# mitschabaude/montgomery

Hardware: AMD Instinct MI355X
Metric: BLS12-377 G1 MSM throughput (higher is better)
Workload: dtype u32

## Files before the change

montgomery_amd/csrc/msm_sort.hip:

```cpp
#include "msm_internal.h"

using namespace msm;
using namespace msmi;

namespace msmi {

void sort_kernel_attributes() {
  HIPCHK(hipFuncSetAttribute((const void*)k_hist, hipFuncAttributeMaxDynamicSharedMemorySize, 128 * 1024));
  HIPCHK(hipFuncSetAttribute((const void*)k_scatter_lds, hipFuncAttributeMaxDynamicSharedMemorySize, 128 * 1024));
  HIPCHK(hipFuncSetAttribute((const void*)k_bin_split, hipFuncAttributeMaxDynamicSharedMemorySize, (int)bin_split_lds(1u << BS_MAX_AB)));
  HIPCHK(hipFuncSetAttribute((const void*)k_bin_pairs, hipFuncAttributeMaxDynamicSharedMemorySize, (int)bin_pairs_lds(1u << BS_MAX_FB)));
  HIPCHK(hipFuncSetAttribute((const void*)k_bin_slots, hipFuncAttributeMaxDynamicSharedMemorySize, (int)bin_slots_lds(1u << BS_MAX_FB)));
  const int dig_lds = 16 * (1 << BS_MAX_AB) * 4;
#define MSM_DIGITS_ATTR(ID, CV) HIPCHK(hipFuncSetAttribute((const void*)k_digits<CV>, hipFuncAttributeMaxDynamicSharedMemorySize, dig_lds));
  MSM_W_CURVES(MSM_DIGITS_ATTR)
#undef MSM_DIGITS_ATTR
  HIPCHK(hipFuncSetAttribute((const void*)te::k_te_digits, hipFuncAttributeMaxDynamicSharedMemorySize, dig_lds));
#define MSM_NARROW_ATTR(W)                                                                                                    \
  HIPCHK(hipFuncSetAttribute((const void*)k_digits_narrow<W>, hipFuncAttributeMaxDynamicSharedMemorySize, dig_lds));          \
  HIPCHK(hipFuncSetAttribute((const void*)k_te_digits_narrow<W>, hipFuncAttributeMaxDynamicSharedMemorySize, dig_lds));
  MSM_NARROW_WIDTHS(MSM_NARROW_ATTR)
#undef MSM_NARROW_ATTR
}

// ... 124 lines not shown
  } else if (radix && cuts) {
    if (kc > 16) throw MsmFail{MSM_ERR_INTERNAL, "more than 16 windows in a radix-split group"};
    for (int kk = 0; kk < kc; kk++) { ws.ab[kk] = (uint8_t)(cbits - (int)RX_FINE_BITS); ws.fb[kk] = (uint8_t)RX_FINE_BITS; }
  }
  const uint32_t Hn = radix ? 1u << (cbits - (int)RX_FINE_BITS) : 1u;
  const uint32_t V = (uint32_t)kc * (bin_split ? hb : Hn);
  uint32_t sortB = 1;
  uint64_t chunk = two_n, pps = n;
  if (bin_split) {
    const uint64_t mult = 4;
    sortB = (uint32_t)std::max<uint64_t>(1, std::min<uint64_t>((uint64_t)mult * ctx->n_cu, n / 4096));
    const uint64_t max_pps = (1ull << BS_SPAN_LOG) / (te ? 1 : 2);
    sortB = (uint32_t)std::max<uint64_t>(sortB, (n + max_pps - 1) / max_pps);
    pps = (n + sortB - 1) / sortB;
    chunk = (te ? 1 : 2) * pps;
    if (consume) {
      if (share->sortB != sortB || share->pps != pps || share->chunk != chunk || share->hb < hb)
        throw MsmFail{MSM_ERR_INTERNAL, "shared digits do not match the group's sort geometry"};
      hb = share->hb;
    } else {
      ctx->ensure(w.block_hist, (size_t)kc_d * sortB * hb * 4 + 64);
    }
  } else {
    const uint64_t mult = two_n >= (1ull << 27) ? 8 : two_n >= (1ull << 24) ? 4 : 2;
    uint64_t want = std::max<uint64_t>(1, (mult * ctx->n_cu + kc - 1) / kc);
    uint64_t maxb = std::max<uint64_t>(1, two_n / 8192);
    sortB = (uint32_t)std::min<uint64_t>(want, maxb);
    chunk = (two_n + sortB - 1) / sortB;
    if (!produce) ctx->ensure(w.block_hist, (size_t)kc * sortB * L * 4 + 64);
  }
  uint32_t* d_bin_start = nullptr;
  uint32_t *d_extra_first = nullptr, *d_mp_first = nullptr, *d_part_pair_off = nullptr;
  uint32_t part_len = 0, part_grid = 0;
  bool will_chunk = false;
  {
    const int chunk_rows_log = ctx->chunk_rows_log;
    const uint64_t table_rows = pl.tables ? (uint64_t)kc_d * n : n;
    const bool want_chunks = bin_split && !te && pl.c >= 18 && table_rows > (1ull << chunk_rows_log);
    will_chunk = bin_split && want_chunks && !te && logG >= 2;
  }
  if (produce && !bin_split && !digits_only) return;
  if (produce) ctx->ensure(w.dig, n_entries * 4);
  if (share && !share->produce && !bin_split) throw MsmFail{MSM_ERR_INTERNAL, "shared digits for a group that does not take the bin split"};
  const uint32_t* dig_p = consume ? share->dig + (uint64_t)(k_lo - share->k_lo) * two_n_d : (const uint32_t*)w.dig.p;
  uint32_t* hist_p = consume ? share->hist + (uint64_t)(k_lo - share->k_lo) * sortB * hb : (uint32_t*)w.block_hist.p;

  if (consume) HIPCHK(hipStreamWaitEvent(s, share->ready, 0));
  HIPCHK(hipEventRecord(w.ev[0], s));
  if (pl.nar.width) {
    if (!consume) narrow_digits(ctx, w, d_scalars, n, pl, k_lo, kc_d, bin_split, radix, sortB, pps, hb, ws, digits_only);
  } else if (pl.batch) {
    if (((bin_split || radix) && !digits_only) || k_lo != 0 || kc_d != pl.batch * pl.K) throw MsmFail{MSM_ERR_INTERNAL, "a batch group outside the one-level sort"};
    const uint32_t grid = (uint32_t)((n + 255) / 256);
    if (te)
      hipLaunchKernelGGL(te::k_te_digits_batch, dim3(grid), dim3(256), 0, s, (uint32_t*)w.dig.p, pl.batch_sc, (uint32_t)pl.batch,
                         (uint32_t)n, pl.c, pl.K, pl.strict ? 1 : 0, (uint32_t*)ctx->errflag.p);
    else
      W_LAUNCH(ctx, k_digits_batch, dim3(grid), dim3(256), 0, s, (uint32_t*)w.dig.p, pl.batch_sc, (uint32_t)pl.batch, (uint32_t)n, pl.c,
               pl.K, (pl.no_glv ? 0 : 1) | (pl.fold ? 2 : 0), pl.strict ? 1 : 0, (uint32_t*)ctx->errflag.p);
  } else if (!consume) {
    const uint32_t grid = bin_split ? sortB : (uint32_t)((n + 255) / 256);
    const uint32_t per = bin_split ? (uint32_t)pps : 256u;
    uint32_t* hist = bin_split ? (uint32_t*)w.block_hist.p : nullptr;
    const size_t lds = bin_split ? (size_t)kc_d * hb * 4 : 0;
    WinSplit ws_d = ws;
    if (pl.tables) for (int kk = 0; kk < 16; kk++) ws_d.fb[kk] = ws.fb[0];
    const uint32_t threads = bin_split ? 1024u : 256u;
    if (te)
      hipLaunchKernelGGL(te::k_te_digits, dim3(grid), dim3(threads), lds, s, (uint32_t*)w.dig.p, d_scalars, (uint32_t)n, pl.c, pl.K,
                         k_lo, kc_d, pl.strict ? 1 : 0, (uint32_t*)ctx->errflag.p, per, hist, hb, pack_fine_bits(ws_d), pl.b_lo, pl.b_n, pl.bt_lo, pl.bt_n);
    else
      W_LAUNCH(ctx, k_digits, dim3(grid), dim3(threads), lds, s, (uint32_t*)w.dig.p, d_scalars, (uint32_t)n, pl.c, pl.K, k_lo, kc_d,
                         (pl.no_glv ? 0 : 1) | (pl.fold ? 2 : 0), pl.strict ? 1 : 0, (uint32_t*)ctx->errflag.p, per, hist, hb, pack_fine_bits(ws_d), pl.b_lo, pl.b_n, pl.bt_lo, pl.bt_n);
  }
  if (produce) {
    share->k_lo = k_lo;
    share->dig = (const uint32_t*)w.dig.p;
    share->hist = (uint32_t*)w.block_hist.p;
    share->hb = hb;
    share->sortB = sortB;
    share->pps = pps;
    share->chunk = chunk;
    HIPCHK(hipEventRecord(share->ready, s));
    share->valid = true;
    return;
  }
  HIPCHK(hipEventRecord(w.ev[1], s));
  if (!bin_split) {
    hipLaunchKernelGGL(k_hist, dim3(sortB, kc), dim3(SORT_THREADS), (size_t)L * 4, s, (uint32_t*)w.block_hist.p,
                       (const uint32_t*)w.dig.p, two_n, chunk, L);
    hipLaunchKernelGGL(k_colscan, dim3((uint32_t)((nb + 255) / 256)), dim3(256), 0, s, (uint32_t*)w.block_hist.p,
                       (uint32_t*)w.counts.p, sortB, L, (uint32_t)kc);
  } else {
    ctx->ensure(w.part, ((size_t)2 * V + 2) * 4);
    uint32_t* d_bin_tot = (uint32_t*)w.part.p;
    d_bin_start = d_bin_tot + V;
    ctx->ensure(w.rec, n_entries * 8);
    hipLaunchKernelGGL(k_slice_scan, dim3((hb + 31) / 32, kc), dim3(1024), 0, s, hist_p, d_bin_tot,
                       pl.tables ? sortB * (uint32_t)kc_d : sortB, hb, (uint32_t)kc);
    part_len = (uint32_t)std::max<uint64_t>(1u << 16, ((2 * n_entries / V + BP_TILE - 1) / BP_TILE) * BP_TILE);
    part_grid = V + V / 2 + 1;
    ctx->ensure(w.parts, ((size_t)2 * (V + 1) + (V + 2)) * 4);
    d_extra_first = (uint32_t*)w.parts.p;
    d_mp_first = d_extra_first + (V + 1);
    d_part_pair_off = d_mp_first + (V + 1);
    PartTables ptab{d_extra_first, d_mp_first, d_part_pair_off, hb, part_len, {}};
    for (int kk = 0; kk < 16; kk++) ptab.fb[kk] = ws.fb[kk];
    hipLaunchKernelGGL(k_vscan, dim3(1), dim3(SCAN_THREADS), 0, s, d_bin_start, (const uint32_t*)d_bin_tot, V, (uint32_t*)w.info.p, ptab);
    const uint32_t per_block = (uint32_t)std::min<uint64_t>(std::min<uint64_t>(sortB, std::max<uint64_t>(1, (1ull << BS_SPAN_LOG) / chunk)),
                                                            std::max<uint64_t>(1, (2 * (uint64_t)BS_TILE + chunk - 1) / chunk));
    hipLaunchKernelGGL(k_bin_split, dim3((sortB + per_block - 1) / per_block, kc_d), dim3(BS_THREADS), bin_split_lds(hb), s, (uint2*)w.rec.p,
                       (const uint32_t*)d_bin_start, (const uint32_t*)hist_p, dig_p, two_n_d, chunk, hb, ws,
                       pl.tables ? 1u : 0u, sortB, per_block);
    bool spans_all = true;
    for (int kk = 0; kk < kc; kk++) spans_all &= (1u << ws.ab[kk]) == hb && (int)ws.ab[kk] + (int)ws.fb[kk] == cbits;
    if (!spans_all) HIPCHK(hipMemsetAsync(w.counts.p, 0, nb * 4, s));
    ctx->ensure(w.sub, (size_t)(V + 2) * nbmax * 4);
    hipLaunchKernelGGL(k_bin_count, dim3(part_grid), dim3(BC_THREADS), (size_t)nbmax * 4, s, (uint32_t*)w.counts.p, (const uint32_t*)d_bin_start,
                       (const uint2*)w.rec.p, hb, L, ws, (uint32_t*)w.info.p, V, (const uint32_t*)d_extra_first, (const uint32_t*)d_mp_first,
                       part_len, (uint32_t*)w.sub.p, nbmax);
    hipLaunchKernelGGL(k_part_scan, dim3(V), dim3(PSC_THREADS), 0, s, (uint32_t*)w.counts.p, (uint32_t*)w.sub.p, d_part_pair_off,
                       (const uint32_t*)d_extra_first, (const uint32_t*)d_mp_first, hb, L, nbmax, ws, (uint32_t*)w.info.p,
                       will_chunk ? 1u : 0u);
  }
  scan_bucket_sizes(ctx, w, nb, logG, !bin_split);
  const uint32_t* round1_slots = nullptr;
  const uint32_t* round1_dest = nullptr;
  uint64_t rec_y_off = 0;
  bool chunked = will_chunk;
  const uint64_t parts_extra = will_chunk ? std::min<uint64_t>(n_entries, (uint64_t)V * nbmax) : 0;
  const uint64_t slots_bound = n_entries + parts_extra + (((uint64_t)1 << logG) - 1) * std::min<uint64_t>(nb, n_entries);
  auto launch_bin_pass = [&](uint64_t slots_cap) {
    if (chunked) {
      const uint64_t pairs_cap = slots_cap / 2 + 1;
      ctx->ensure(w.slots2, pairs_cap * 8);
      ctx->ensure(w.dest, pairs_cap * 4);
      rec_y_off = (pairs_cap * 64 + 255) & ~(uint64_t)255;
      ctx->ensure(w.rows1, 2 * rec_y_off + 256);
      hipLaunchKernelGGL(k_bin_pairs, dim3(part_grid), dim3(BP_THREADS), bin_pairs_lds(nbmax), s, (uint2*)w.slots2.p, (uint32_t*)w.dest.p,
                         (const uint2*)w.rec.p, (const uint32_t*)d_bin_start, (const uint32_t*)w.cursor.p, hb, L, nbmax, ws, V,
                         (const uint32_t*)d_extra_first, (const uint32_t*)d_mp_first, part_len, (const uint32_t*)w.sub.p,
                         (const uint32_t*)d_part_pair_off);
      round1_slots = (const uint32_t*)w.slots2.p;
      round1_dest = (const uint32_t*)w.dest.p;
    } else {
      ctx->ensure(w.slots, std::max<uint64_t>(slots_cap, 2) * 4);
      HIPCHK(hipMemsetAsync(w.slots.p, 0xFF, std::max<uint64_t>(slots_cap, 2) * 4, s));
      round1_slots = (const uint32_t*)w.slots.p;
      hipLaunchKernelGGL(k_bin_slots, dim3(part_grid), dim3(BP_THREADS), bin_slots_lds(nbmax), s, (uint32_t*)w.slots.p,
                         (const uint2*)w.rec.p, (const uint32_t*)d_bin_start, (const uint32_t*)w.cursor.p, hb, L, nbmax, ws, V,
                         (const uint32_t*)d_extra_first, (const uint32_t*)d_mp_first, part_len, (const uint32_t*)w.sub.p);
    }
  };
  if (bin_split) launch_bin_pass(slots_bound);
  const ScanTotals tot = read_scan_totals(w, logG);
  const int RT = tot.RT;
  const uint64_t total_slots = tot.total_slots;
  const uint32_t max_bucket = tot.max_bucket;
  st.n_pairs_algo += tot.algo_pairs;
  st.max_bucket = std::max<uint64_t>(st.max_bucket, max_bucket);
  if (total_slots > slots_bound) throw MsmFail{MSM_ERR_INTERNAL, "the padded slots exceed their bound"};
  if (bin_split && chunked && total_slots < 2) {
    chunked = false;
    round1_dest = nullptr;
    rec_y_off = 0;
    launch_bin_pass(2);
  }
  if (!bin_split) {
    ctx->ensure(w.slots, std::max<uint64_t>(total_slots, 2) * 4);
    HIPCHK(hipMemsetAsync(w.slots.p, 0xFF, std::max<uint64_t>(total_slots, 2) * 4, s));
    round1_slots = (const uint32_t*)w.slots.p;
    const bool heavy = radix && max_bucket >= (1u << 16) && (uint64_t)max_bucket * Hn >= 16 * two_n;
    if (radix && !heavy) {
      ctx->ensure(w.part, ((size_t)kc * sortB * Hn + 2 * (size_t)V + 2) * 4);
      uint32_t* d_blk_off = (uint32_t*)w.part.p;
      uint32_t* d_vtot = d_blk_off + (size_t)kc * sortB * Hn;
      uint32_t* d_vstart = d_vtot + V;
      ctx->ensure(w.dig2, n_entries * 4);
      ctx->ensure(w.idx2, n_entries * 4);
      const uint64_t co = (uint64_t)kc * (sortB + 1) * Hn;
      hipLaunchKernelGGL(k_coarse_offsets, dim3((uint32_t)((co + 255) / 256)), dim3(256), 0, s, d_blk_off, d_vtot,
                         (const uint32_t*)w.block_hist.p, (const uint32_t*)w.counts.p, sortB, L, Hn, (uint32_t)kc);
      hipLaunchKernelGGL(k_vscan, dim3(1), dim3(SCAN_THREADS), 0, s, d_vstart, (const uint32_t*)d_vtot, V, (uint32_t*)nullptr, PartTables{});
      hipLaunchKernelGGL(k_radix_coarse, dim3(sortB, kc), dim3(RX_THREADS), 0, s, (uint32_t*)w.dig2.p, (uint32_t*)w.idx2.p,
// ... 23 lines not shown
```

montgomery_amd/csrc/sort_kernels.h:

```cpp
#pragma once
#include "msm_kernels.h"

namespace msm {


constexpr int SCAN_THREADS = 1024;
constexpr int SCAN_ITEMS = 4;

__device__ __forceinline__ void lds_barrier() {
#if defined(__HIP_DEVICE_COMPILE__)
  asm volatile("s_waitcnt lgkmcnt(0)\n\ts_barrier" ::: "memory");
#endif
}

template <bool LDS_ONLY = false>
MSM_DEV uint32_t block_excl_scan(uint32_t v, uint32_t* lds_wave, uint32_t& total) {
  uint32_t x = v;
  const int lane = threadIdx.x & 63, wave = threadIdx.x >> 6;
#pragma unroll
  for (int d = 1; d < 64; d <<= 1) {
    uint32_t y = __shfl_up(x, d, 64);
    if (lane >= d) x += y;
  }
  if (LDS_ONLY) lds_barrier(); else __syncthreads();
// ... 492 lines not shown
      uint32_t v[8];
#pragma unroll
      for (int i = 0; i < 8; i++) v[i] = p[(uint64_t)(b + i) * L];
#pragma unroll
      for (int i = 0; i < 8; i++) sum += v[i];
    }
    for (; b < b1; b++) sum += p[(uint64_t)b * L];
  }
  part[r][c] = sum;
  __syncthreads();
  uint32_t run = 0;
  for (uint32_t q = 0; q < r; q++) run += part[q][c];
  if (live) {
    uint32_t b = b0;
    for (; b + 8 <= b1; b += 8) {
      uint32_t v[8];
#pragma unroll
      for (int i = 0; i < 8; i++) v[i] = p[(uint64_t)(b + i) * L];
#pragma unroll
      for (int i = 0; i < 8; i++) { p[(uint64_t)(b + i) * L] = run; run += v[i]; }
    }
    for (; b < b1; b++) {
      const uint32_t v = p[(uint64_t)b * L];
      p[(uint64_t)b * L] = run;
      run += v;
    }
    if (r == 31) totals[(uint64_t)kk * L + l] = run;
  }
}
#endif

constexpr uint32_t BS_MAX_AB = 11, BS_MAX_FB = 12;
constexpr uint32_t BS_SPAN_LOG = 17;
inline size_t bin_split_lds(uint32_t hb) { return (size_t)BS_TILE * 4 + (size_t)3 * hb * 4 + 64 * 4; }

__global__ void __launch_bounds__(BS_THREADS) k_bin_split(uint2* rec, const uint32_t* bin_start, const uint32_t* slice_off,
                                                          const uint32_t* dig, uint64_t two_n, uint64_t chunk, uint32_t hb, WinSplit ws,
                                                          uint32_t merged, uint32_t SBd, uint32_t g)
#ifndef MSM_SORT_TU
    ;
#else
{
  extern __shared__ uint32_t lds_bs[];
  uint32_t* stage = lds_bs;
  uint32_t* t_cnt = stage + BS_TILE;
  uint32_t* t_start = t_cnt + hb;
  uint32_t* g_base = t_start + hb;
  uint32_t* lds_wave = g_base + hb;
  const uint32_t b = blockIdx.x, seg = blockIdx.y, tid = threadIdx.x;
  const uint32_t kk = merged ? 0u : seg;
  const uint32_t ab = ws.ab[kk], fb = ws.fb[kk], HN = 1u << ab;
  for (uint32_t h = tid; h < HN; h += BS_THREADS)
    g_base[h] = bin_start[(uint64_t)kk * hb + h] + slice_off[((uint64_t)seg * SBd + (uint64_t)b * g) * hb + h];
  const uint64_t beg = (uint64_t)b * g * chunk, end = min(beg + (uint64_t)g * chunk, two_n);
  const uint32_t* d = dig + (uint64_t)seg * two_n;
  const uint32_t e_first = (merged ? (uint32_t)((uint64_t)seg * two_n) : 0u) + (uint32_t)beg;
  const uint32_t fmask = (1u << fb) - 1;
  uint32_t v[BS_ITEMS];
  auto load_tile = [&](uint64_t t0) {
#if defined(__HIP_DEVICE_COMPILE__)
    const uint32_t left = t0 < end ? (uint32_t)min<uint64_t>(end - t0, BS_TILE) : 0u;
    const uint64_t a = (uint64_t)(d + t0);
    const uint32_t a_lo = __builtin_amdgcn_readfirstlane((uint32_t)a), a_hi = __builtin_amdgcn_readfirstlane((uint32_t)(a >> 32));
    const auto rs = __builtin_amdgcn_make_buffer_rsrc((void*)(((uint64_t)a_hi << 32) | a_lo), 0, __builtin_amdgcn_readfirstlane(left * 4u), 0x00020000);
#pragma unroll
    for (int i = 0; i < BS_ITEMS; i++) v[i] = (uint32_t)__builtin_amdgcn_raw_buffer_load_b32(rs, tid * 4u, i * BS_THREADS * 4, 0);
#endif
  };
  load_tile(beg);
  for (uint64_t t0 = beg; t0 < end; t0 += BS_TILE) {
    for (uint32_t h = tid; h < HN; h += BS_THREADS) t_cnt[h] = 0;
    lds_barrier();
    uint32_t rk[BS_ITEMS / 2];
#pragma unroll
    for (int i = 0; i < BS_ITEMS; i++) {
      const uint32_t l = v[i] & 0x7FFFFFFFu;
      const uint32_t r = lds_rank_add(t_cnt, l ? (l - 1) >> fb : 0u, l != 0);
      if (i & 1) rk[i / 2] |= r << 16; else rk[i / 2] = r;
#if defined(__HIP_DEVICE_COMPILE__)
      if ((i & 7) == 7) __builtin_amdgcn_sched_barrier(0);
#endif
    }
    lds_barrier();
    (void)bucket_scan<BS_THREADS, true>(HN, lds_wave, [&](uint32_t h) { return t_cnt[h]; }, [&](uint32_t h, uint32_t ex) { t_start[h] = ex; });
    lds_barrier();
#if defined(__HIP_DEVICE_COMPILE__)
#pragma unroll
    for (int i = 0; i < BS_ITEMS; i++) asm volatile("" : "+v"(v[i]));
#endif
    const uint32_t off0 = (uint32_t)(t0 - beg) + tid;
#pragma unroll
    for (int i = 0; i < BS_ITEMS; i++) {
      const uint32_t l = v[i] & 0x7FFFFFFFu;
      if (l) stage[t_start[(l - 1) >> fb] + ((rk[i / 2] >> (16 * (i & 1))) & 0xFFFFu)] = (((l - 1) & fmask) + 1) | ((off0 + (uint32_t)i * BS_THREADS) << 13) | (v[i] & 0x80000000u);
#if defined(__HIP_DEVICE_COMPILE__)
      if ((i & 7) == 7) __builtin_amdgcn_sched_barrier(0);
#endif
    }
    lds_barrier();
    load_tile(t0 + BS_TILE);
    const uint32_t lane = tid & 31u;
    for (uint32_t h = tid >> 5; h < HN; h += BS_THREADS / 32) {
      const uint32_t T = t_cnt[h], pos = g_base[h], ts = t_start[h];
      for (uint32_t o = lane; o < T; o += 32) {
        const uint32_t r = stage[ts + o];
        rec[pos + o] = make_uint2(r & 0x80001FFFu, e_first + ((r >> 13) & ((1u << BS_SPAN_LOG) - 1)));
      }
      if (lane == 0) g_base[h] = pos + T;
    }
    lds_barrier();
  }
}
#endif

struct PartLoc {
  uint32_t v, j, np, row;
  uint64_t beg, end;
  bool valid;
};
__device__ __forceinline__ PartLoc locate_part(uint32_t p, uint32_t V, const uint32_t* bin_start, const uint32_t* extra_first,
                                               const uint32_t* mp_first, uint32_t part_len, bool reverse) {
  PartLoc L;
  L.valid = true;
  if (p < V) {
    L.v = reverse ? V - 1 - p : p;
    L.j = 0;
  } else {
    const uint32_t q = p - V;
    if (q >= extra_first[V]) { L.valid = false; L.v = L.j = L.np = L.row = 0; L.beg = L.end = 0; return L; }
    uint32_t lo = 0, hi = V;
    while (hi - lo > 1) {
      const uint32_t mid = (lo + hi) >> 1;
      if (extra_first[mid] <= q) lo = mid; else hi = mid;
    }
    L.v = lo;
    L.j = 1 + q - extra_first[lo];
  }
  L.np = extra_first[L.v + 1] - extra_first[L.v] + 1;
  L.row = mp_first[L.v] + L.j;
  const uint64_t b0 = bin_start[L.v], b1 = bin_start[L.v + 1];
// ... 47 lines not shown
#pragma unroll
  for (int i = 0; i < IT; i++) {
    const uint32_t bk = tid + i * PSC_THREADS;
    if (bk < NB) {
      const uint32_t cnt = pairs_mode ? 2 * run[i] : tot[i];
      out[bk] = cnt;
      mx = max(mx, cnt);
      sum += tot[i] ? tot[i] - 1 : 0;
    }
  }
  for (int o = 32; o > 0; o >>= 1) { sum += __shfl_down(sum, o); mx = max(mx, (uint32_t)__shfl_down(mx, o)); }
  if ((tid & 63u) == 0 && (mx | sum)) { atomicMax(&lds_max, mx); atomicAdd(&lds_sum, sum); }
  __threadfence();
  __syncthreads();
  if (tid == 0) {
    atomicMax(&info[1], lds_max);
    atomicAdd(reinterpret_cast<unsigned long long*>(info + INFO_ALGO_PAIRS), lds_sum);
  }
  if (!pairs_mode) return;
  uint32_t carry = 0;
  for (uint32_t base = 0; base < np; base += PSC_THREADS) {
    const uint32_t j = base + tid;
    const uint32_t x = j < np ? __hip_atomic_load(&part_pair_off[row0 + j], __ATOMIC_RELAXED, __HIP_MEMORY_SCOPE_AGENT) : 0u;
    uint32_t t;
    const uint32_t ex = block_excl_scan(x, lds_wave, t) + carry;
    __syncthreads();
    if (j < np) part_pair_off[row0 + j] = ex;
    carry += t;
  }
}
#endif

constexpr int BC_THREADS = 1024;
__global__ void __launch_bounds__(BC_THREADS) k_bin_count(uint32_t* counts, const uint32_t* bin_start, const uint2* rec, uint32_t hb, uint32_t L,
                                                          WinSplit ws, uint32_t* info, uint32_t V, const uint32_t* extra_first,
                                                          const uint32_t* mp_first, uint32_t part_len, uint32_t* sub, uint32_t nbmax)
#ifndef MSM_SORT_TU
    ;
#else
{
  extern __shared__ uint32_t lds_bc[];
  __shared__ uint32_t lds_max;
  __shared__ unsigned long long lds_sum;
  const uint32_t tid = threadIdx.x;
  const PartLoc pl = locate_part(blockIdx.x, V, bin_start, extra_first, mp_first, part_len, false);
  if (!pl.valid) return;
  const uint32_t v = pl.v;
  const uint32_t kk = v / hb, h = v - kk * hb, fb = ws.fb[kk], NB = 1u << fb;
  if (h >= (1u << ws.ab[kk])) return;
  const uint64_t beg = pl.beg, end = pl.end;
  uint32_t* out = counts + (uint64_t)kk * L + ((uint64_t)h << fb);
  if (beg == end) {
    for (uint32_t j = tid; j < NB; j += BC_THREADS) out[j] = 0;
    return;
  }
  if (fb == 0) {
    if (tid == 0) {
      out[0] = (uint32_t)(end - beg);
      atomicMax(&info[1], (uint32_t)(end - beg));
      atomicAdd(reinterpret_cast<unsigned long long*>(info + INFO_ALGO_PAIRS), (unsigned long long)(end - beg - 1));
    }
    return;
  }
  if (tid == 0) { lds_max = 0; lds_sum = 0; }
  for (uint32_t j = tid; j < NB; j += BC_THREADS) lds_bc[j] = 0;
  __syncthreads();
  const uint4* rec2 = reinterpret_cast<const uint4*>(rec);
  for (uint64_t j0 = beg >> 1; 2 * j0 < end; j0 += BC_THREADS) {
    const uint64_t j = j0 + tid;
    uint4 r = make_uint4(0, 0, 0, 0);
    if (2 * j < end) r = rec2[j];
    const uint32_t l0 = (2 * j >= beg && 2 * j < end) ? r.x & 0xFFFFu : 0u;
    const uint32_t l1 = (2 * j + 1 >= beg && 2 * j + 1 < end) ? r.z & 0xFFFFu : 0u;
    (void)lds_rank_add(lds_bc, l0 ? l0 - 1 : 0u, l0 != 0);
    (void)lds_rank_add(lds_bc, l1 ? l1 - 1 : 0u, l1 != 0);
  }
  __syncthreads();
  if (pl.np > 1) {
    uint32_t* row = sub + (uint64_t)pl.row * nbmax;
    for (uint32_t j = tid; j < NB; j += BC_THREADS) row[j] = lds_bc[j];
    return;
  }
  uint32_t mx = 0;
  unsigned long long sum = 0;
  for (uint32_t j = tid; j < NB; j += BC_THREADS) {
    const uint32_t cnt = lds_bc[j];
    out[j] = cnt;
    mx = max(mx, cnt);
    sum += cnt ? cnt - 1 : 0;
  }
  for (int o = 32; o > 0; o >>= 1) { sum += __shfl_down(sum, o); mx = max(mx, (uint32_t)__shfl_down(mx, o)); }
  if ((tid & 63u) == 0 && (mx | sum)) { atomicMax(&lds_max, mx); atomicAdd(&lds_sum, sum); }
  __syncthreads();
  if (tid == 0) {
    atomicMax(&info[1], lds_max);
    atomicAdd(reinterpret_cast<unsigned long long*>(info + INFO_ALGO_PAIRS), lds_sum);
  }
}
#endif

constexpr int BP_THREADS = 512, BP_ITEMS = 8, BP_TILE = BP_THREADS * BP_ITEMS;
inline size_t bin_pairs_lds(uint32_t nbmax) { return (size_t)5 * nbmax * 4 + 64 * 4 + (size_t)((BP_TILE + nbmax) / 2 + 1) * 12; }
inline size_t bin_slots_lds(uint32_t nbmax) { return (size_t)3 * nbmax * 4 + 64 * 4 + (size_t)BP_TILE * 6; }

__global__ void __launch_bounds__(BP_THREADS) k_bin_pairs(uint2* pairs, uint32_t* dest, const uint2* rec, const uint32_t* bin_start,
                                                          const uint32_t* cursor, uint32_t hb, uint32_t L, uint32_t nbmax, WinSplit ws,
                                                          uint32_t V, const uint32_t* extra_first, const uint32_t* mp_first,
                                                          uint32_t part_len, const uint32_t* sub, const uint32_t* part_pair_off)
#ifndef MSM_SORT_TU
    ;
#else
{
  extern __shared__ uint32_t lds_bp[];
  const uint32_t st_cap = (BP_TILE + nbmax) / 2 + 1;
  uint2* st_pair = reinterpret_cast<uint2*>(lds_bp);
  uint32_t* st_dest = lds_bp + 2 * st_cap;
  uint32_t* t_cnt = st_dest + st_cap;
  uint32_t* p_start = t_cnt + nbmax;
  uint32_t* t_delta = p_start + nbmax;
  uint32_t* pend = t_delta + nbmax;
  uint32_t* g_next = pend + nbmax;
  uint32_t* lds_wave = g_next + nbmax;
  const uint32_t tid = threadIdx.x;
  const PartLoc pl = locate_part(blockIdx.x, V, bin_start, extra_first, mp_first, part_len, true);
  if (!pl.valid) return;
  const uint32_t v = pl.v;
  const uint32_t kk = v / hb, h = v - kk * hb;
  const uint32_t ab = ws.ab[kk], fb = ws.fb[kk], NB = 1u << fb, HN = 1u << ab;
  const uint32_t* cur = cursor + (uint64_t)kk * L;
  if (fb == 0) {
    const uint32_t* bs = bin_start + (uint64_t)kk * hb;
    const uint64_t d0 = cur[0] >> 1, d1 = cur[HN] >> 1, len = d1 - d0;
    const uint64_t beg = d0 + len * h / hb, end = d0 + len * (h + 1) / hb;
    for (uint64_t dd = beg + tid; dd < end; dd += BP_THREADS) {
      uint32_t lo = 0, hi = HN;
      while (hi - lo > 1) {
        const uint32_t mid = (lo + hi) >> 1;
        if ((cur[mid] >> 1) <= dd) lo = mid; else hi = mid;
      }
      const uint32_t q = (uint32_t)(dd - (cur[lo] >> 1)), nent = bs[lo + 1] - bs[lo];
      const uint64_t r0 = (uint64_t)bs[lo] + 2ull * q;
      uint2 pr = make_uint2(SLOT_EMPTY, SLOT_EMPTY);
      if (2 * q < nent) { const uint2 r = rec[r0]; pr.x = (r.y << 1) | (r.x >> 31); }
      if (2 * q + 1 < nent) { const uint2 r = rec[r0 + 1]; pr.y = (r.y << 1) | (r.x >> 31); }
      pairs[dd] = pr;
      dest[dd] = (uint32_t)dd;
    }
    return;
  }
  if (h >= HN) return;
  const uint32_t* curb = cur + ((uint64_t)h << fb);
  const uint64_t beg = pl.beg, end = pl.end;
  if (beg == end) return;
  const uint32_t* sub_row = pl.np > 1 ? sub + (uint64_t)pl.row * nbmax : nullptr;
  for (uint32_t bk = tid; bk < NB; bk += BP_THREADS) {
    pend[bk] = SLOT_EMPTY;
    g_next[bk] = (curb[bk] >> 1) + (sub_row ? sub_row[bk] : 0u);
  }
  uint64_t out_pos = (curb[0] >> 1) + (sub_row ? part_pair_off[pl.row] : 0u);
  uint2 r[BP_ITEMS], nr[BP_ITEMS];
  auto load_tile = [&](uint2 (&dst)[BP_ITEMS], uint64_t t0) {
#pragma unroll
    for (int i = 0; i < BP_ITEMS; i++) {
      const uint64_t j = t0 + (uint64_t)i * BP_THREADS + tid;
      dst[i] = j < end ? rec[j] : make_uint2(0u, 0u);
    }
  };
  load_tile(r, beg);
  for (uint64_t t0 = beg; t0 < end; t0 += BP_TILE) {
    for (uint32_t bk = tid; bk < NB; bk += BP_THREADS) t_cnt[bk] = 0;
    lds_barrier();
    uint32_t rk[BP_ITEMS];
#pragma unroll
    for (int i = 0; i < BP_ITEMS; i++) {
      const uint32_t l = r[i].x & 0xFFFFu;
      rk[i] = lds_rank_add(t_cnt, l ? l - 1 : 0u, l != 0);
    }
    load_tile(nr, t0 + BP_TILE);
    __syncthreads();
    const uint32_t n_pairs = bucket_scan<BP_THREADS>(
        NB, lds_wave, [&](uint32_t bk) { return ((pend[bk] != SLOT_EMPTY ? 1u : 0u) + t_cnt[bk]) >> 1; },
        [&](uint32_t bk, uint32_t ex) {
          const uint32_t has = pend[bk] != SLOT_EMPTY ? 1u : 0u, m = has + t_cnt[bk], np = m >> 1;
          p_start[bk] = ex | (has << 31);
          t_delta[bk] = g_next[bk] - ex;
          g_next[bk] += np;
          if (has && np) {
            st_pair[ex].x = pend[bk];
            st_dest[ex] = t_delta[bk] + ex;
            pend[bk] = SLOT_EMPTY;
          }
        });
    __syncthreads();
#pragma unroll
    for (int i = 0; i < BP_ITEMS; i++) {
      const uint32_t l = r[i].x & 0xFFFFu;
      if (l) {
        const uint32_t bk = l - 1, ps = p_start[bk], has = ps >> 31, m = has + t_cnt[bk], sq = rk[i] + has;
        const uint32_t payload = (r[i].y << 1) | (r[i].x >> 31);
        if ((m & 1u) && sq == m - 1) pend[bk] = payload;
        else {
          const uint32_t p = (ps & 0x7FFFFFFFu) + (sq >> 1);
          if (sq & 1u) st_pair[p].y = payload;
          else { st_pair[p].x = payload; st_dest[p] = t_delta[bk] + p; }
        }
      }
    }
    __syncthreads();
    for (uint32_t p = tid; p < n_pairs; p += BP_THREADS) {
      pairs[out_pos + p] = st_pair[p];
      dest[out_pos + p] = st_dest[p];
    }
    out_pos += n_pairs;
    __syncthreads();
#pragma unroll
    for (int i = 0; i < BP_ITEMS; i++) r[i] = nr[i];
  }
  if (pl.j + 1 < pl.np) {
    (void)bucket_scan<BP_THREADS>(
        NB, lds_wave, [&](uint32_t bk) { return pend[bk] != SLOT_EMPTY ? 1u : 0u; },
        [&](uint32_t bk, uint32_t ex) {
          if (pend[bk] != SLOT_EMPTY) {
            pairs[out_pos + ex] = make_uint2(pend[bk], SLOT_EMPTY);
            dest[out_pos + ex] = g_next[bk];
          }
        });
    return;
  }
  (void)bucket_scan<BP_THREADS>(
      NB, lds_wave, [&](uint32_t bk) { return (curb[bk + 1] >> 1) - g_next[bk]; },
      [&](uint32_t bk, uint32_t ex) {
        const uint32_t rem = (curb[bk + 1] >> 1) - g_next[bk];
        for (uint32_t j = 0; j < rem; j++) {
          pairs[out_pos + ex + j] = make_uint2(j == 0 ? pend[bk] : SLOT_EMPTY, SLOT_EMPTY);
          dest[out_pos + ex + j] = g_next[bk] + j;
        }
      });
}
#endif

__global__ void __launch_bounds__(BP_THREADS) k_bin_slots(uint32_t* slots, const uint2* rec, const uint32_t* bin_start,
                                                          const uint32_t* cursor, uint32_t hb, uint32_t L, uint32_t nbmax, WinSplit ws,
                                                          uint32_t V, const uint32_t* extra_first, const uint32_t* mp_first,
                                                          uint32_t part_len, const uint32_t* sub)
#ifndef MSM_SORT_TU
    ;
#else
{
  extern __shared__ uint32_t lds_bp[];
  uint32_t* t_cnt = lds_bp;
  uint32_t* t_start = t_cnt + nbmax;
  uint32_t* g_cur = t_start + nbmax;
  uint32_t* lds_wave = g_cur + nbmax;
  uint32_t* stage = lds_wave + 64;
  uint16_t* stage_b = reinterpret_cast<uint16_t*>(stage + BP_TILE);
  const uint32_t tid = threadIdx.x;
  const PartLoc pl = locate_part(blockIdx.x, V, bin_start, extra_first, mp_first, part_len, true);
  if (!pl.valid) return;
  const uint32_t v = pl.v;
  const uint32_t kk = v / hb, h = v - kk * hb;
  const uint32_t ab = ws.ab[kk], fb = ws.fb[kk], NB = 1u << fb, HN = 1u << ab;
  const uint32_t* cur = cursor + (uint64_t)kk * L;
  if (fb == 0) {
    const uint32_t* bs = bin_start + (uint64_t)kk * hb;
    const uint64_t wbeg = bs[0], wlen = (uint64_t)bs[HN] - wbeg;
    const uint64_t beg = wbeg + wlen * h / hb, end = wbeg + wlen * (h + 1) / hb;
    for (uint64_t j = beg + tid; j < end; j += BP_THREADS) {
      uint32_t lo = 0, hi = HN;
      while (hi - lo > 1) {
        const uint32_t mid = (lo + hi) >> 1;
        if (bs[mid] <= j) lo = mid; else hi = mid;
      }
      const uint2 r = rec[j];
      slots[cur[lo] + (uint32_t)(j - bs[lo])] = (r.y << 1) | (r.x >> 31);
    }
    return;
  }
  if (h >= HN) return;
  const uint64_t beg = pl.beg, end = pl.end;
  if (beg == end) return;
  const uint32_t* sub_row = pl.np > 1 ? sub + (uint64_t)pl.row * nbmax : nullptr;
  for (uint32_t bk = tid; bk < NB; bk += BP_THREADS) g_cur[bk] = cur[((uint64_t)h << fb) + bk] + (sub_row ? sub_row[bk] : 0u);
  for (uint64_t t0 = beg; t0 < end; t0 += BP_TILE) {
    for (uint32_t bk = tid; bk < NB; bk += BP_THREADS) t_cnt[bk] = 0;
    lds_barrier();
    uint2 r[BP_ITEMS];
    uint32_t rk[BP_ITEMS];
#pragma unroll
    for (int i = 0; i < BP_ITEMS; i++) {
      const uint64_t j = t0 + (uint64_t)i * BP_THREADS + tid;
      r[i] = j < end ? rec[j] : make_uint2(0u, 0u);
    }
#pragma unroll
    for (int i = 0; i < BP_ITEMS; i++) {
      const uint32_t l = r[i].x & 0xFFFFu;
      rk[i] = lds_rank_add(t_cnt, l ? l - 1 : 0u, l != 0);
    }
    lds_barrier();
    const uint32_t n_tile = bucket_scan<BP_THREADS, true>(NB, lds_wave, [&](uint32_t bk) { return t_cnt[bk]; },
                                           [&](uint32_t bk, uint32_t ex) { t_start[bk] = ex; });
    lds_barrier();
#pragma unroll
    for (int i = 0; i < BP_ITEMS; i++) {
      const uint32_t l = r[i].x & 0xFFFFu;
      if (l) {
        const uint32_t p = t_start[l - 1] + rk[i];
        stage[p] = (r[i].y << 1) | (r[i].x >> 31);
        stage_b[p] = (uint16_t)(l - 1);
      }
    }
    lds_barrier();
    for (uint32_t i = tid; i < n_tile; i += BP_THREADS) {
      const uint32_t bk = stage_b[i];
      slots[g_cur[bk] + (i - t_start[bk])] = stage[i];
    }
    lds_barrier();
    for (uint32_t bk = tid; bk < NB; bk += BP_THREADS) g_cur[bk] += t_cnt[bk];
  }
}
#endif

}
```

Baseline: 524.4 million.

## Pack bin-split records into 32 bits and reconstruct entry index from run offsets

The bin-split intermediate record shrinks from a uint2 (fine bucket plus full entry index) to a single uint32 holding the fine bucket, a span-local offset and the sign bit. Downstream kernels (bin_count, bin_pairs, bin_slots) rebuild the global entry index by locating the source run through the per-slice histogram offsets, using an LDS window of run starts with per-64-record granule bounds. This halves the global write and read traffic on the record array. In exchange it adds LDS, extra barriers and binary searches to the pairing and slot kernels, plus more complex indexing logic.

```diff
diff --git a/montgomery_amd/csrc/msm_sort.hip b/montgomery_amd/csrc/msm_sort.hip
--- a/montgomery_amd/csrc/msm_sort.hip
+++ b/montgomery_amd/csrc/msm_sort.hip
@@ -180,6 +180,7 @@
   uint32_t* d_bin_start = nullptr;
   uint32_t *d_extra_first = nullptr, *d_mp_first = nullptr, *d_part_pair_off = nullptr;
   uint32_t part_len = 0, part_grid = 0;
+  BinRuns bin_runs{};
   bool will_chunk = false;
   {
     const int chunk_rows_log = ctx->chunk_rows_log;
@@ -243,7 +244,7 @@
     ctx->ensure(w.part, ((size_t)2 * V + 2) * 4);
     uint32_t* d_bin_tot = (uint32_t*)w.part.p;
     d_bin_start = d_bin_tot + V;
-    ctx->ensure(w.rec, n_entries * 8);
+    ctx->ensure(w.rec, n_entries * 4);
     hipLaunchKernelGGL(k_slice_scan, dim3((hb + 31) / 32, kc), dim3(1024), 0, s, hist_p, d_bin_tot,
                        pl.tables ? sortB * (uint32_t)kc_d : sortB, hb, (uint32_t)kc);
     part_len = (uint32_t)std::max<uint64_t>(1u << 16, ((2 * n_entries / V + BP_TILE - 1) / BP_TILE) * BP_TILE);
@@ -257,15 +258,18 @@
     hipLaunchKernelGGL(k_vscan, dim3(1), dim3(SCAN_THREADS), 0, s, d_bin_start, (const uint32_t*)d_bin_tot, V, (uint32_t*)w.info.p, ptab);
     const uint32_t per_block = (uint32_t)std::min<uint64_t>(std::min<uint64_t>(sortB, std::max<uint64_t>(1, (1ull << BS_SPAN_LOG) / chunk)),
                                                             std::max<uint64_t>(1, (2 * (uint64_t)BS_TILE + chunk - 1) / chunk));
-    hipLaunchKernelGGL(k_bin_split, dim3((sortB + per_block - 1) / per_block, kc_d), dim3(BS_THREADS), bin_split_lds(hb), s, (uint2*)w.rec.p,
+    const uint32_t nblk = (sortB + per_block - 1) / per_block;
+    hipLaunchKernelGGL(k_bin_split, dim3(nblk, kc_d), dim3(BS_THREADS), bin_split_lds(hb), s, (uint32_t*)w.rec.p,
                        (const uint32_t*)d_bin_start, (const uint32_t*)hist_p, dig_p, two_n_d, chunk, hb, ws,
                        pl.tables ? 1u : 0u, sortB, per_block);
+    bin_runs = BinRuns{(const uint32_t*)hist_p, sortB, per_block, nblk, pl.tables ? (uint32_t)kc_d * nblk : nblk,
+                       pl.tables ? (uint32_t)two_n_d : 0u, (uint32_t)chunk};
     bool spans_all = true;
     for (int kk = 0; kk < kc; kk++) spans_all &= (1u << ws.ab[kk]) == hb && (int)ws.ab[kk] + (int)ws.fb[kk] == cbits;
     if (!spans_all) HIPCHK(hipMemsetAsync(w.counts.p, 0, nb * 4, s));
     ctx->ensure(w.sub, (size_t)(V + 2) * nbmax * 4);
     hipLaunchKernelGGL(k_bin_count, dim3(part_grid), dim3(BC_THREADS), (size_t)nbmax * 4, s, (uint32_t*)w.counts.p, (const uint32_t*)d_bin_start,
-                       (const uint2*)w.rec.p, hb, L, ws, (uint32_t*)w.info.p, V, (const uint32_t*)d_extra_first, (const uint32_t*)d_mp_first,
+                       (const uint32_t*)w.rec.p, hb, L, ws, (uint32_t*)w.info.p, V, (const uint32_t*)d_extra_first, (const uint32_t*)d_mp_first,
                        part_len, (uint32_t*)w.sub.p, nbmax);
     hipLaunchKernelGGL(k_part_scan, dim3(V), dim3(PSC_THREADS), 0, s, (uint32_t*)w.counts.p, (uint32_t*)w.sub.p, d_part_pair_off,
                        (const uint32_t*)d_extra_first, (const uint32_t*)d_mp_first, hb, L, nbmax, ws, (uint32_t*)w.info.p,
@@ -286,9 +290,9 @@
       rec_y_off = (pairs_cap * 64 + 255) & ~(uint64_t)255;
       ctx->ensure(w.rows1, 2 * rec_y_off + 256);
       hipLaunchKernelGGL(k_bin_pairs, dim3(part_grid), dim3(BP_THREADS), bin_pairs_lds(nbmax), s, (uint2*)w.slots2.p, (uint32_t*)w.dest.p,
-                         (const uint2*)w.rec.p, (const uint32_t*)d_bin_start, (const uint32_t*)w.cursor.p, hb, L, nbmax, ws, V,
+                         (const uint32_t*)w.rec.p, (const uint32_t*)d_bin_start, (const uint32_t*)w.cursor.p, hb, L, nbmax, ws, V,
                          (const uint32_t*)d_extra_first, (const uint32_t*)d_mp_first, part_len, (const uint32_t*)w.sub.p,
-                         (const uint32_t*)d_part_pair_off);
+                         (const uint32_t*)d_part_pair_off, bin_runs);
       round1_slots = (const uint32_t*)w.slots2.p;
       round1_dest = (const uint32_t*)w.dest.p;
     } else {
@@ -296,8 +300,8 @@
       HIPCHK(hipMemsetAsync(w.slots.p, 0xFF, std::max<uint64_t>(slots_cap, 2) * 4, s));
       round1_slots = (const uint32_t*)w.slots.p;
       hipLaunchKernelGGL(k_bin_slots, dim3(part_grid), dim3(BP_THREADS), bin_slots_lds(nbmax), s, (uint32_t*)w.slots.p,
-                         (const uint2*)w.rec.p, (const uint32_t*)d_bin_start, (const uint32_t*)w.cursor.p, hb, L, nbmax, ws, V,
-                         (const uint32_t*)d_extra_first, (const uint32_t*)d_mp_first, part_len, (const uint32_t*)w.sub.p);
+                         (const uint32_t*)w.rec.p, (const uint32_t*)d_bin_start, (const uint32_t*)w.cursor.p, hb, L, nbmax, ws, V,
+                         (const uint32_t*)d_extra_first, (const uint32_t*)d_mp_first, part_len, (const uint32_t*)w.sub.p, bin_runs);
     }
   };
   if (bin_split) launch_bin_pass(slots_bound);
diff --git a/montgomery_amd/csrc/sort_kernels.h b/montgomery_amd/csrc/sort_kernels.h
--- a/montgomery_amd/csrc/sort_kernels.h
+++ b/montgomery_amd/csrc/sort_kernels.h
@@ -548,9 +548,115 @@
 
 constexpr uint32_t BS_MAX_AB = 11, BS_MAX_FB = 12;
 constexpr uint32_t BS_SPAN_LOG = 17;
+constexpr uint32_t BS_REC_FINE_BITS = BS_MAX_FB + 1, BS_REC_FINE_MASK = (1u << BS_REC_FINE_BITS) - 1;
+constexpr uint32_t BS_REC_OFF_MASK = (1u << BS_SPAN_LOG) - 1, BS_REC_SIGN = 0x80000000u;
+static_assert((1u << BS_MAX_FB) <= BS_REC_FINE_MASK && BS_REC_FINE_BITS + BS_SPAN_LOG <= 31, "a bin-split record must fit 32 bits");
 inline size_t bin_split_lds(uint32_t hb) { return (size_t)BS_TILE * 4 + (size_t)3 * hb * 4 + 64 * 4; }
 
-__global__ void __launch_bounds__(BS_THREADS) k_bin_split(uint2* rec, const uint32_t* bin_start, const uint32_t* slice_off,
+struct BinRuns {
+  const uint32_t* slice_off;
+  uint32_t SBd, g, nblk;
+  uint32_t n_runs;
+  uint32_t seg_entries;
+  uint32_t chunk;
+};
+constexpr uint32_t BR_NONE = 0xFFFFFFFFu;
+__device__ __forceinline__ uint32_t bin_run(const BinRuns& R, uint32_t kk, uint32_t hb, uint32_t h, uint32_t r, uint32_t& e_first) {
+  const uint32_t seg = r / R.nblk, b = r - seg * R.nblk;
+  e_first = seg * R.seg_entries + b * R.g * R.chunk;
+  if (r >= R.n_runs) return BR_NONE;
+  return R.slice_off[((uint64_t)(kk + seg) * R.SBd + (uint64_t)b * R.g) * hb + h];
+}
+__device__ __forceinline__ uint32_t bin_run_of(const BinRuns& R, uint32_t kk, uint32_t hb, uint32_t h, uint32_t p) {
+  uint32_t lo = 0, hi = R.n_runs, e;
+  while (hi - lo > 1) {
+    const uint32_t mid = (lo + hi) >> 1;
+    if (bin_run(R, kk, hb, h, mid, e) <= p) lo = mid; else hi = mid;
+  }
+  return lo;
+}
+__device__ __forceinline__ uint32_t bin_record_entry(const BinRuns& R, uint32_t kk, uint32_t hb, uint32_t h, uint32_t p, uint32_t rec) {
+  uint32_t e;
+  (void)bin_run(R, kk, hb, h, bin_run_of(R, kk, hb, h, p), e);
+  return e + ((rec >> BS_REC_FINE_BITS) & BS_REC_OFF_MASK);
+}
+
+constexpr uint32_t BR_WIN = 256, BR_GRAN_MAX = 72;
+inline size_t bin_runs_lds() { return (size_t)(2 * BR_WIN + BR_GRAN_MAX) * 4; }
+struct RunWindow {
+  uint32_t* start;
+  uint32_t* first;
+  uint32_t* gran;
+  uint32_t base;
+  uint32_t kk, hb, h;
+  uint32_t nxt_s;
+  __device__ __forceinline__ void init(uint32_t* lds) { start = lds; first = lds + BR_WIN; gran = first + BR_WIN; }
+  __device__ __forceinline__ void prefetch(const BinRuns& R) {
+    uint32_t e;
+    if (threadIdx.x < BR_WIN) nxt_s = bin_run(R, kk, hb, h, base + (BR_WIN - 1) + threadIdx.x, e);
+  }
+  __device__ __forceinline__ void load(const BinRuns& R) {
+    if (threadIdx.x < BR_WIN) {
+      uint32_t e;
+      start[threadIdx.x] = bin_run(R, kk, hb, h, base + threadIdx.x, e);
+      first[threadIdx.x] = e;
+    }
+    prefetch(R);
+  }
+  template <int THREADS, int ITEMS>
+  __device__ __forceinline__ void prepare(uint32_t tile0, uint32_t p_last) {
+    constexpr uint32_t G = ITEMS * (THREADS / 64);
+    static_assert(G + 1 <= BR_GRAN_MAX && G + 1 <= THREADS && BR_WIN <= THREADS, "one thread per 64 records of the tile");
+    const uint32_t t = THREADS - 1 - threadIdx.x;
+    if (t <= G) gran[t] = slot_of(min(tile0 + t * 64u, p_last));
+  }
+  __device__ __forceinline__ uint32_t slot_of(uint32_t p) const {
+    uint32_t idx = 0;
+#pragma unroll
+    for (uint32_t step = BR_WIN / 2; step; step >>= 1) idx += start[idx + step] <= p ? step : 0u;
+    return idx;
+  }
+  template <int THREADS, int ITEMS>
+  __device__ __forceinline__ void resolve(const BinRuns& R, uint32_t (&rec)[ITEMS], uint32_t p0, uint32_t p_last) {
+    constexpr uint32_t WAVES = THREADS / 64;
+    const uint32_t tid = threadIdx.x, wave = tid >> 6;
+    for (;;) {
+      const uint32_t lo_v = start[0], hi_v = start[BR_WIN - 1];
+      const bool whole = lo_v <= p0 - tid && p_last < hi_v;
+#pragma unroll
+      for (int i = 0; i < ITEMS; i++) {
+        const uint32_t p = p0 + (uint32_t)i * THREADS, g = (uint32_t)i * WAVES + wave;
+        uint32_t lo = gran[g], n = gran[g + 1] - lo;
+#if defined(__HIP_DEVICE_COMPILE__)
+        lo = __builtin_amdgcn_readfirstlane(lo);
+        n = __builtin_amdgcn_readfirstlane(n);
+#endif
+        uint32_t idx = lo;
+        if (n == 1) idx += start[lo + 1] <= p ? 1u : 0u;
+        else if (n) {
+          for (uint32_t step = 1u << (31 - __builtin_clz(n)); step; step >>= 1)
+            if (idx + step <= lo + n && start[idx + step] <= p) idx += step;
+        }
+        const uint32_t payload = ((first[idx] + ((rec[i] >> BS_REC_FINE_BITS) & BS_REC_OFF_MASK)) << 1) | (rec[i] >> 31);
+        if (whole || (rec[i] && p >= lo_v && p < hi_v)) rec[i] = payload;
+      }
+      if (p_last < hi_v) return;
+      __syncthreads();
+      base += BR_WIN - 1;
+      if (tid < BR_WIN) {
+        const uint32_t r = base + tid, seg = r / R.nblk;
+        start[tid] = nxt_s;
+        first[tid] = seg * R.seg_entries + (r - seg * R.nblk) * R.g * R.chunk;
+      }
+      prefetch(R);
+      __syncthreads();
+      prepare<THREADS, ITEMS>(p0 - tid, p_last);
+      __syncthreads();
+    }
+  }
+};
+
+__global__ void __launch_bounds__(BS_THREADS) k_bin_split(uint32_t* rec, const uint32_t* bin_start, const uint32_t* slice_off,
                                                           const uint32_t* dig, uint64_t two_n, uint64_t chunk, uint32_t hb, WinSplit ws,
                                                           uint32_t merged, uint32_t SBd, uint32_t g)
 #ifndef MSM_SORT_TU
@@ -570,7 +676,6 @@
     g_base[h] = bin_start[(uint64_t)kk * hb + h] + slice_off[((uint64_t)seg * SBd + (uint64_t)b * g) * hb + h];
   const uint64_t beg = (uint64_t)b * g * chunk, end = min(beg + (uint64_t)g * chunk, two_n);
   const uint32_t* d = dig + (uint64_t)seg * two_n;
-  const uint32_t e_first = (merged ? (uint32_t)((uint64_t)seg * two_n) : 0u) + (uint32_t)beg;
   const uint32_t fmask = (1u << fb) - 1;
   uint32_t v[BS_ITEMS];
   auto load_tile = [&](uint64_t t0) {
@@ -608,7 +713,7 @@
 #pragma unroll
     for (int i = 0; i < BS_ITEMS; i++) {
       const uint32_t l = v[i] & 0x7FFFFFFFu;
-      if (l) stage[t_start[(l - 1) >> fb] + ((rk[i / 2] >> (16 * (i & 1))) & 0xFFFFu)] = (((l - 1) & fmask) + 1) | ((off0 + (uint32_t)i * BS_THREADS) << 13) | (v[i] & 0x80000000u);
+      if (l) stage[t_start[(l - 1) >> fb] + ((rk[i / 2] >> (16 * (i & 1))) & 0xFFFFu)] = (((l - 1) & fmask) + 1) | ((off0 + (uint32_t)i * BS_THREADS) << BS_REC_FINE_BITS) | (v[i] & BS_REC_SIGN);
 #if defined(__HIP_DEVICE_COMPILE__)
       if ((i & 7) == 7) __builtin_amdgcn_sched_barrier(0);
 #endif
@@ -618,10 +723,7 @@
     const uint32_t lane = tid & 31u;
     for (uint32_t h = tid >> 5; h < HN; h += BS_THREADS / 32) {
       const uint32_t T = t_cnt[h], pos = g_base[h], ts = t_start[h];
-      for (uint32_t o = lane; o < T; o += 32) {
-        const uint32_t r = stage[ts + o];
-        rec[pos + o] = make_uint2(r & 0x80001FFFu, e_first + ((r >> 13) & ((1u << BS_SPAN_LOG) - 1)));
-      }
+      for (uint32_t o = lane; o < T; o += 32) rec[pos + o] = stage[ts + o];
       if (lane == 0) g_base[h] = pos + T;
     }
     lds_barrier();
@@ -735,7 +837,7 @@
 #endif
 
 constexpr int BC_THREADS = 1024;
-__global__ void __launch_bounds__(BC_THREADS) k_bin_count(uint32_t* counts, const uint32_t* bin_start, const uint2* rec, uint32_t hb, uint32_t L,
+__global__ void __launch_bounds__(BC_THREADS) k_bin_count(uint32_t* counts, const uint32_t* bin_start, const uint32_t* rec, uint32_t hb, uint32_t L,
                                                           WinSplit ws, uint32_t* info, uint32_t V, const uint32_t* extra_first,
                                                           const uint32_t* mp_first, uint32_t part_len, uint32_t* sub, uint32_t nbmax)
 #ifndef MSM_SORT_TU
@@ -768,15 +870,17 @@
   if (tid == 0) { lds_max = 0; lds_sum = 0; }
   for (uint32_t j = tid; j < NB; j += BC_THREADS) lds_bc[j] = 0;
   __syncthreads();
-  const uint4* rec2 = reinterpret_cast<const uint4*>(rec);
-  for (uint64_t j0 = beg >> 1; 2 * j0 < end; j0 += BC_THREADS) {
+  const uint4* rec4 = reinterpret_cast<const uint4*>(rec);
+  for (uint64_t j0 = beg >> 2; 4 * j0 < end; j0 += BC_THREADS) {
     const uint64_t j = j0 + tid;
     uint4 r = make_uint4(0, 0, 0, 0);
-    if (2 * j < end) r = rec2[j];
-    const uint32_t l0 = (2 * j >= beg && 2 * j < end) ? r.x & 0xFFFFu : 0u;
-    const uint32_t l1 = (2 * j + 1 >= beg && 2 * j + 1 < end) ? r.z & 0xFFFFu : 0u;
-    (void)lds_rank_add(lds_bc, l0 ? l0 - 1 : 0u, l0 != 0);
-    (void)lds_rank_add(lds_bc, l1 ? l1 - 1 : 0u, l1 != 0);
+    if (4 * j < end) r = rec4[j];
+    const uint32_t w[4] = {r.x, r.y, r.z, r.w};
+#pragma unroll
+    for (int q = 0; q < 4; q++) {
+      const uint32_t l = (4 * j + q >= beg && 4 * j + q < end) ? w[q] & BS_REC_FINE_MASK : 0u;
+      (void)lds_rank_add(lds_bc, l ? l - 1 : 0u, l != 0);
+    }
   }
   __syncthreads();
   if (pl.np > 1) {
@@ -803,13 +907,13 @@
 #endif
 
 constexpr int BP_THREADS = 512, BP_ITEMS = 8, BP_TILE = BP_THREADS * BP_ITEMS;
-inline size_t bin_pairs_lds(uint32_t nbmax) { return (size_t)5 * nbmax * 4 + 64 * 4 + (size_t)((BP_TILE + nbmax) / 2 + 1) * 12; }
-inline size_t bin_slots_lds(uint32_t nbmax) { return (size_t)3 * nbmax * 4 + 64 * 4 + (size_t)BP_TILE * 6; }
-
-__global__ void __launch_bounds__(BP_THREADS) k_bin_pairs(uint2* pairs, uint32_t* dest, const uint2* rec, const uint32_t* bin_start,
+inline size_t bin_pairs_lds(uint32_t nbmax) { return (size_t)5 * nbmax * 4 + 64 * 4 + (size_t)((BP_TILE + nbmax) / 2 + 1) * 12 + bin_runs_lds(); }
+inline size_t bin_slots_lds(uint32_t nbmax) { return (size_t)3 * nbmax * 4 + 64 * 4 + (size_t)BP_TILE * 6 + bin_runs_lds(); }
+
+__global__ void __launch_bounds__(BP_THREADS) k_bin_pairs(uint2* pairs, uint32_t* dest, const uint32_t* rec, const uint32_t* bin_start,
                                                           const uint32_t* cursor, uint32_t hb, uint32_t L, uint32_t nbmax, WinSplit ws,
                                                           uint32_t V, const uint32_t* extra_first, const uint32_t* mp_first,
-                                                          uint32_t part_len, const uint32_t* sub, const uint32_t* part_pair_off)
+                                                          uint32_t part_len, const uint32_t* sub, const uint32_t* part_pair_off, BinRuns runs)
 #ifndef MSM_SORT_TU
     ;
 #else
@@ -824,6 +928,8 @@
   uint32_t* pend = t_delta + nbmax;
   uint32_t* g_next = pend + nbmax;
   uint32_t* lds_wave = g_next + nbmax;
+  RunWindow rw;
+  rw.init(lds_wave + 64);
   const uint32_t tid = threadIdx.x;
   const PartLoc pl = locate_part(blockIdx.x, V, bin_start, extra_first, mp_first, part_len, true);
   if (!pl.valid) return;
@@ -844,8 +950,8 @@
       const uint32_t q = (uint32_t)(dd - (cur[lo] >> 1)), nent = bs[lo + 1] - bs[lo];
       const uint64_t r0 = (uint64_t)bs[lo] + 2ull * q;
       uint2 pr = make_uint2(SLOT_EMPTY, SLOT_EMPTY);
-      if (2 * q < nent) { const uint2 r = rec[r0]; pr.x = (r.y << 1) | (r.x >> 31); }
-      if (2 * q + 1 < nent) { const uint2 r = rec[r0 + 1]; pr.y = (r.y << 1) | (r.x >> 31); }
+      if (2 * q < nent) { const uint32_t r = rec[r0]; pr.x = (bin_record_entry(runs, kk, hb, lo, 2 * q, r) << 1) | (r >> 31); }
+      if (2 * q + 1 < nent) { const uint32_t r = rec[r0 + 1]; pr.y = (bin_record_entry(runs, kk, hb, lo, 2 * q + 1, r) << 1) | (r >> 31); }
       pairs[dd] = pr;
       dest[dd] = (uint32_t)dd;
     }
@@ -861,23 +967,32 @@
     g_next[bk] = (curb[bk] >> 1) + (sub_row ? sub_row[bk] : 0u);
   }
   uint64_t out_pos = (curb[0] >> 1) + (sub_row ? part_pair_off[pl.row] : 0u);
-  uint2 r[BP_ITEMS], nr[BP_ITEMS];
-  auto load_tile = [&](uint2 (&dst)[BP_ITEMS], uint64_t t0) {
+  const uint32_t bin_beg = bin_start[v];
+  rw.kk = kk; rw.hb = hb; rw.h = h;
+  rw.base = pl.j ? bin_run_of(runs, kk, hb, h, (uint32_t)(beg - bin_beg)) : 0u;
+  rw.load(runs);
+  uint32_t r[BP_ITEMS], nr[BP_ITEMS];
+  auto load_tile = [&](uint32_t (&dst)[BP_ITEMS], uint64_t t0) {
+    const uint32_t* rt = rec + t0;
+    const uint32_t left = t0 < end ? (uint32_t)min<uint64_t>(end - t0, BP_TILE) : 0u;
 #pragma unroll
     for (int i = 0; i < BP_ITEMS; i++) {
-      const uint64_t j = t0 + (uint64_t)i * BP_THREADS + tid;
-      dst[i] = j < end ? rec[j] : make_uint2(0u, 0u);
+      const uint32_t o = (uint32_t)i * BP_THREADS + tid;
+      dst[i] = o < left ? rt[o] : 0u;
     }
   };
   load_tile(r, beg);
+  __syncthreads();
   for (uint64_t t0 = beg; t0 < end; t0 += BP_TILE) {
+    const uint32_t tile0 = (uint32_t)(t0 - bin_beg), p_last = (uint32_t)(min<uint64_t>(t0 + BP_TILE, end) - 1 - bin_beg);
     for (uint32_t bk = tid; bk < NB; bk += BP_THREADS) t_cnt[bk] = 0;
+    rw.prepare<BP_THREADS, BP_ITEMS>(tile0, p_last);
     lds_barrier();
     uint32_t rk[BP_ITEMS];
 #pragma unroll
     for (int i = 0; i < BP_ITEMS; i++) {
-      const uint32_t l = r[i].x & 0xFFFFu;
-      rk[i] = lds_rank_add(t_cnt, l ? l - 1 : 0u, l != 0);
+      const uint32_t l = r[i] & BS_REC_FINE_MASK;
+      rk[i] = lds_rank_add(t_cnt, l ? l - 1 : 0u, l != 0) | (l << 16);
     }
     load_tile(nr, t0 + BP_TILE);
     __syncthreads();
@@ -895,12 +1010,13 @@
           }
         });
     __syncthreads();
+    rw.resolve<BP_THREADS>(runs, r, tile0 + tid, p_last);
 #pragma unroll
     for (int i = 0; i < BP_ITEMS; i++) {
-      const uint32_t l = r[i].x & 0xFFFFu;
+      const uint32_t l = rk[i] >> 16;
       if (l) {
-        const uint32_t bk = l - 1, ps = p_start[bk], has = ps >> 31, m = has + t_cnt[bk], sq = rk[i] + has;
-        const uint32_t payload = (r[i].y << 1) | (r[i].x >> 31);
+        const uint32_t bk = l - 1, ps = p_start[bk], has = ps >> 31, m = has + t_cnt[bk], sq = (rk[i] & 0xFFFFu) + has;
+        const uint32_t payload = r[i];
         if ((m & 1u) && sq == m - 1) pend[bk] = payload;
         else {
           const uint32_t p = (ps & 0x7FFFFFFFu) + (sq >> 1);
@@ -942,10 +1058,10 @@
 }
 #endif
 
-__global__ void __launch_bounds__(BP_THREADS) k_bin_slots(uint32_t* slots, const uint2* rec, const uint32_t* bin_start,
+__global__ void __launch_bounds__(BP_THREADS) k_bin_slots(uint32_t* slots, const uint32_t* rec, const uint32_t* bin_start,
                                                           const uint32_t* cursor, uint32_t hb, uint32_t L, uint32_t nbmax, WinSplit ws,
                                                           uint32_t V, const uint32_t* extra_first, const uint32_t* mp_first,
-                                                          uint32_t part_len, const uint32_t* sub)
+                                                          uint32_t part_len, const uint32_t* sub, BinRuns runs)
 #ifndef MSM_SORT_TU
     ;
 #else
@@ -957,6 +1073,8 @@
   uint32_t* lds_wave = g_cur + nbmax;
   uint32_t* stage = lds_wave + 64;
   uint16_t* stage_b = reinterpret_cast<uint16_t*>(stage + BP_TILE);
+  RunWindow rw;
+  rw.init(reinterpret_cast<uint32_t*>(stage_b + BP_TILE));
   const uint32_t tid = threadIdx.x;
   const PartLoc pl = locate_part(blockIdx.x, V, bin_start, extra_first, mp_first, part_len, true);
   if (!pl.valid) return;
@@ -974,8 +1092,8 @@
         const uint32_t mid = (lo + hi) >> 1;
         if (bs[mid] <= j) lo = mid; else hi = mid;
       }
-      const uint2 r = rec[j];
-      slots[cur[lo] + (uint32_t)(j - bs[lo])] = (r.y << 1) | (r.x >> 31);
+      const uint32_t r = rec[j], p = (uint32_t)(j - bs[lo]);
+      slots[cur[lo] + p] = (bin_record_entry(runs, kk, hb, lo, p, r) << 1) | (r >> 31);
     }
     return;
   }
@@ -984,31 +1102,38 @@
   if (beg == end) return;
   const uint32_t* sub_row = pl.np > 1 ? sub + (uint64_t)pl.row * nbmax : nullptr;
   for (uint32_t bk = tid; bk < NB; bk += BP_THREADS) g_cur[bk] = cur[((uint64_t)h << fb) + bk] + (sub_row ? sub_row[bk] : 0u);
+  const uint32_t bin_beg = bin_start[v];
+  rw.kk = kk; rw.hb = hb; rw.h = h;
+  rw.base = pl.j ? bin_run_of(runs, kk, hb, h, (uint32_t)(beg - bin_beg)) : 0u;
+  rw.load(runs);
+  __syncthreads();
   for (uint64_t t0 = beg; t0 < end; t0 += BP_TILE) {
+    const uint32_t tile0 = (uint32_t)(t0 - bin_beg), p_last = (uint32_t)(min<uint64_t>(t0 + BP_TILE, end) - 1 - bin_beg);
     for (uint32_t bk = tid; bk < NB; bk += BP_THREADS) t_cnt[bk] = 0;
+    rw.prepare<BP_THREADS, BP_ITEMS>(tile0, p_last);
     lds_barrier();
-    uint2 r[BP_ITEMS];
-    uint32_t rk[BP_ITEMS];
+    uint32_t r[BP_ITEMS], rk[BP_ITEMS];
 #pragma unroll
     for (int i = 0; i < BP_ITEMS; i++) {
       const uint64_t j = t0 + (uint64_t)i * BP_THREADS + tid;
-      r[i] = j < end ? rec[j] : make_uint2(0u, 0u);
+      r[i] = j < end ? rec[j] : 0u;
     }
 #pragma unroll
     for (int i = 0; i < BP_ITEMS; i++) {
-      const uint32_t l = r[i].x & 0xFFFFu;
-      rk[i] = lds_rank_add(t_cnt, l ? l - 1 : 0u, l != 0);
+      const uint32_t l = r[i] & BS_REC_FINE_MASK;
+      rk[i] = lds_rank_add(t_cnt, l ? l - 1 : 0u, l != 0) | (l << 16);
     }
     lds_barrier();
+    rw.resolve<BP_THREADS>(runs, r, tile0 + tid, p_last);
     const uint32_t n_tile = bucket_scan<BP_THREADS, true>(NB, lds_wave, [&](uint32_t bk) { return t_cnt[bk]; },
                                            [&](uint32_t bk, uint32_t ex) { t_start[bk] = ex; });
     lds_barrier();
 #pragma unroll
     for (int i = 0; i < BP_ITEMS; i++) {
-      const uint32_t l = r[i].x & 0xFFFFu;
+      const uint32_t l = rk[i] >> 16;
       if (l) {
-        const uint32_t p = t_start[l - 1] + rk[i];
-        stage[p] = (r[i].y << 1) | (r[i].x >> 31);
+        const uint32_t p = t_start[l - 1] + (rk[i] & 0xFFFFu);
+        stage[p] = r[i];
         stage_b[p] = (uint16_t)(l - 1);
       }
     }
```

New measurement: 517.6 million. 0.987x the previous value.
